# MoonInTheRiver/DiffSinger

Hardware: NVIDIA H100
Metric: mel-frames/s (higher is better)
Workload: dtype f16 operands (weights stochastically rounded per step), 1 MMA pass, conditioner projection hoisted (f32), f32 accumulate and state

## Files before the change

diffsinger_b200/csrc/dsx_hopper.cu:

```cuda
#include <stdio.h>
#include <string.h>

#include <algorithm>
#include <cmath>
#include <string>
#include <vector>

#include "dsx_internal.h"
#include "dsx_ptx.cuh"
#include "dsx_rng.cuh"

namespace dsx {

constexpr int kC = 256;
constexpr int kRowsPerLayer = 80 * 256;
constexpr int kSrRowsPerLayer = 32 * 256;
constexpr int kWBytes = 256 * 128;
constexpr int kABytes = 64 * 128;
constexpr int kZBytes = 4 * kABytes;
constexpr int kEpiBatch = 8;

constexpr int kHalo = 8;

template <int NWG, int R, bool WIN = (R == 3)>
struct StepCfg {
  static_assert(R == 2 || R == 3, "ring depth");
  static constexpr int THREADS = NWG * 128;
  static constexpr int STAGE = kWBytes + (WIN ? 0 : NWG * kABytes);
  static constexpr int BARS = R * STAGE;
  static constexpr int W = BARS + 1024;
  static constexpr int WROWS = 64 * NWG + 2 * kHalo;
  static constexpr int WBLK = WROWS * 128;
  static constexpr int ZHI23 = 2 * kABytes;
  static constexpr int ASLOT = NWG * ZHI23;
  static constexpr int WSIZE = WIN ? std::max(4 * WBLK, ASLOT + R * NWG * kABytes) : 0;
  static constexpr int ZHI = W + WSIZE;
  static constexpr int ZHI_WG = WIN ? 2 * kABytes : kZBytes;
  static constexpr int ZLO = ZHI + NWG * ZHI_WG;
  static constexpr int SMEM = 1024 + ZLO + NWG * (R == 2 ? kZBytes : kABytes);
  static_assert(WBLK % 1024 == 0 && ASLOT % 1024 == 0, "window blocks and activation slots start 1024-aligned");
  static_assert(!WIN || NWG * ZHI23 <= WSIZE, "z hi k-blocks 2-3 fit in W");
  static_assert(SMEM <= 232448, "shared memory budget (227 KB per block on sm_90)");
};
constexpr int kCondSmem = 1024 + StepCfg<2, 3, false>::BARS + 2 * 3 * 8;

struct HpParams {
  const __half* w;
  int w_sr;
  int P;
  int HP;
  int ylo;
  int fast_gate;
  const __half* whead;
  float* X;
  float* SKIP;
  __half* Y;
  __half* S16;
  const __half* CONDH;
  size_t plane;
  float* CP;
  const float* b1p;
  const float* b2;
  const float* dtab;
  int d_row_stride;
  int T, Tp, B, units;
  int l0, l1, L, cycle;
  float inv_sqrt_l;
  int head_flags;
  float* x;
  dsx_strides xs;
  float* eps;
  const float* noise;
  unsigned long long seed, offset;
  int b_off;
  DdpmCoef c;
  PlmsFuse pl;
  const float* bs;
  const float* bf;
  const float* bin;
  const float* d0;
  int d0_row_stride;
  int M;
  long long* trace;
  int trace_ctas;
  unsigned* flags;
};

__device__ __forceinline__ void stamp(const HpParams& p, int slot) {
  if (p.trace != nullptr && threadIdx.x == 0 && slot < DSX_TRACE_SLOTS && static_cast<int>(blockIdx.x) < p.trace_ctas) {
    long long t;
    asm volatile("mov.u64 %0, %%globaltimer;" : "=l"(t)::"memory");
    p.trace[static_cast<size_t>(blockIdx.x) * DSX_TRACE_SLOTS + slot] = t;
  }
}
__device__ __forceinline__ int layer_slot(const HpParams& p, int l, int k) { return 1 + 9 * (l - p.l0) + k; }
__device__ __forceinline__ int head_slot(const HpParams& p, int k) { return 1 + 9 * (p.l1 - p.l0) + k; }

template <int NWG>
__device__ __forceinline__ int partner_tile(const HpParams& p, int u) {
  if (p.units > static_cast<int>(gridDim.x) || p.B < 2) return -1;
  const int tpu = p.Tp / (64 * NWG), b = u / tpu;
  if (b & 1) return u - tpu;
  return b + 1 < p.B ? u + tpu : -1;
}

template <int NWG>
__device__ __forceinline__ void wait_neighbours(const HpParams& p, int u, unsigned n) {
  const int tpu = p.Tp / (64 * NWG);
  if (u % tpu != 0) wait_geq(p.flags + u - 1, n);
  if ((u + 1) % tpu != 0) wait_geq(p.flags + u + 1, n);
}

template <int NWG>
__device__ __forceinline__ void wait_layer(const HpParams& p, int l, int u) {
  if (threadIdx.x == 0) {
    const unsigned n = l - p.l0;
    if (n > 0) wait_neighbours<NWG>(p, u, n);
    const int pu = partner_tile<NWG>(p, u);
    if (pu >= 0 && pu < u) wait_geq(p.flags + p.units + pu, n + 1);
  }
  __syncthreads();
}

template <int NT>
__device__ __forceinline__ void load_w(uint8_t* dst, const __half* src0, const __half* src1, int nrows, int tid) {
  const uint32_t d = smem_u32(dst);
  for (int i = tid; i < nrows * 8; i += NT) {
    const int r = i >> 3, c = i & 7;
    const __half* src = (r < 128 ? src0 + static_cast<size_t>(r) * 64 : src1 + static_cast<size_t>(r - 128) * 64) + c * 8;
// ... 6 lines not shown
  for (int k = 0; k < 4; ++k) {
    const int i = wtid + k * 128;
    const int r = i >> 3, c = i & 7, t = t0 + r;
    const bool valid = t >= 0 && t < T;
    cp16(d + sw128(r, c), src + (static_cast<size_t>(b) * Tp + (valid ? t : 0)) * kC + ch0 + c * 8, valid);
  }
}
template <int NT>
__device__ __forceinline__ void load_wblock(uint8_t* dst, const __half* utt, int t_first, int ch0, int rows, int T, int tid) {
  const uint32_t d = smem_u32(dst);
#pragma unroll 1
  for (int i = tid; i < rows * 8; i += NT) {
    const int r = i >> 3, c = i & 7, t = t_first + r;
    const bool valid = t >= 0 && t < T;
    cp16_hint(d + sw128(r, c), utt + static_cast<size_t>(valid ? t : 0) * kC + ch0 + c * 8, valid, l2_evict_first());
  }
}

template <int N>
__device__ __forceinline__ void fence_acc(float (&d)[N]) {
#pragma unroll
  for (int i = 0; i < N; ++i) asm volatile("" : "+f"(d[i])::"memory");
}

struct NoPrefetch {
  __device__ __forceinline__ void operator()(int) const {}
};

__device__ __forceinline__ uint8_t* smem_base() {
  extern __shared__ uint8_t smem_raw[];
  return reinterpret_cast<uint8_t*>((reinterpret_cast<uintptr_t>(smem_raw) + 1023) & ~uintptr_t(1023));
}

template <int NWG, int R, bool WIN = (R == 3)>
struct Smem {
  using Cfg = StepCfg<NWG, R, WIN>;
  uint32_t n, nw;
  __device__ __forceinline__ uint8_t* slot(uint32_t i) const { return smem_base() + (i % R) * Cfg::STAGE; }
  __device__ __forceinline__ uint32_t full(uint32_t i) const { return smem_u32(smem_base() + Cfg::BARS) + (i % R) * 8; }
  __device__ __forceinline__ uint32_t empty(uint32_t i) const { return full(i) + R * 8; }
  __device__ __forceinline__ uint32_t parity(uint32_t i) const { return (i / R) & 1; }
  __device__ __forceinline__ uint8_t* wblk(int c) const { return smem_base() + Cfg::W + c * Cfg::WBLK; }
  __device__ __forceinline__ uint32_t wbar(int c) const { return full(0) + 2 * R * 8 + c * 8; }
  __device__ __forceinline__ uint8_t* ablk(int j, int wg) const {
    if (WIN) return smem_base() + Cfg::W + Cfg::ASLOT + j * NWG * kABytes + wg * kABytes;
    return smem_base() + j * Cfg::STAGE + kWBytes + wg * kABytes;
  }
  __device__ __forceinline__ uint8_t* zblk(int plane, int kb) const {
    const int wg = threadIdx.x >> 7;
    if (plane == 0) {
      if (WIN && kb >= 2) return smem_base() + Cfg::W + wg * Cfg::ZHI23 + (kb - 2) * kABytes;
      return smem_base() + Cfg::ZHI + wg * Cfg::ZHI_WG + kb * kABytes;
    }
    if (!WIN) return smem_base() + Cfg::ZLO + wg * kZBytes + kb * kABytes;
    return kb < R ? ablk(kb, wg) : smem_base() + Cfg::ZLO + wg * kABytes;
  }
  __device__ __forceinline__ uint8_t* zat(int plane, int r, int k) const {
    return zblk(plane, k >> 6) + sw128(r, (k & 63) >> 3) + (k & 7) * 2;
  }
  __device__ __forceinline__ void init() {
    n = 0;
    nw = 0;
    if (threadIdx.x == 0) {
      for (int j = 0; j < R; ++j) {
        mbar_init(full(j), 1 + NWG * 128);
        mbar_init(empty(j), NWG);
      }
      if (WIN)
        for (int c = 0; c < 4; ++c) mbar_init(wbar(c), NWG * 128);
      fence_mbar_init();
    }
    __syncthreads();
  }
};

enum PhaseKind { PH_NONE, PH_G1, PH_G2, PH_H1, PH_H2, PH_IN, PH_COND };
struct Phase {
  int kind, l, u, hq;
};
__device__ __forceinline__ Phase head_phase(const HpParams& p, int u) {
  const int kind = u >= p.units ? PH_NONE : (p.head_flags & TC_HEAD) ? PH_H1 : (p.head_flags & TC_INPROJ) ? PH_IN : PH_NONE;
  return Phase{kind, 0, u, 0};
}
__device__ __forceinline__ Phase after_layer(const HpParams& p, int l) {
  const int u0 = blockIdx.x;
  if (l + 1 < p.l1) return Phase{PH_G1, l + 1, u0, 0};
  return p.head_flags ? head_phase(p, u0) : Phase{PH_NONE, 0, 0, 0};
}

struct StageSrc {
  const __half* w0;
  const __half* w1;
  uint32_t wbytes;
  const __half* a;
  int b, at, ach;
  int wrow;
  int zplane, zkb;
};

__device__ __forceinline__ const __half* w1_tile(const HpParams& p, int l, int plane, int h, int kb) {
  if (p.w_sr) return p.w + (static_cast<size_t>(l) * kSrRowsPerLayer + (h * 12 + kb) * 256) * 64;
  return p.w + (static_cast<size_t>(l) * kRowsPerLayer + ((plane * 2 + h) * 16 + kb) * 256) * 64;
}
__device__ __forceinline__ const __half* w2_tile(const HpParams& p, int l, int plane, int q, int kb) {
  if (p.w_sr) return p.w + (static_cast<size_t>(l) * kSrRowsPerLayer + (24 + q * 4 + kb) * 256) * 64;
  return p.w + (static_cast<size_t>(l) * kRowsPerLayer + (64 + (plane * 2 + q) * 4 + kb) * 256) * 64;
}
__device__ __forceinline__ const __half* whead_tile(const HpParams& p, int idx) {
  return p.whead + static_cast<size_t>(idx) * 128 * 64;
}
__device__ __forceinline__ int pass_wplane(int ps) { return ps == 1 ? 1 : 0; }
__device__ __forceinline__ int pass_aplane(int ps) { return ps == 2 ? 1 : 0; }

__device__ __forceinline__ int phase_passes(const HpParams& p, int kind) {
  return kind == PH_COND ? 3 : (kind >= PH_H1 ? p.HP : p.P);
}
__device__ __forceinline__ int phase_stages(const HpParams& p, const Phase& ph) {
  const int kbs = ph.kind == PH_G1 ? 12 : ph.kind == PH_IN ? 2 : ph.kind == PH_NONE ? 0 : 4;
  return kbs * phase_passes(p, ph.kind);
}

template <int NWG, bool WIN>
__device__ __forceinline__ StageSrc stage_src(const HpParams& p, const Phase& ph, int s) {
  const int frame0 = ph.u * 64 * NWG;
  const int P = phase_passes(p, ph.kind);
  const int kb = s / P, ps = s % P, wp = pass_wplane(ps), ap = pass_aplane(ps);
  StageSrc st;
  st.w1 = nullptr;
  st.wbytes = kWBytes;
  st.a = nullptr;
  st.b = frame0 / p.Tp;
  st.at = frame0 % p.Tp + (threadIdx.x >> 7) * 64;
  st.ach = kb * 64;
  st.wrow = -1;
  st.zplane = ap;
  st.zkb = kb;
  switch (ph.kind) {
    case PH_G1: {
      const int shift = ((kb >> 2) - 1) * (1 << (ph.l % p.cycle));
      st.w0 = w1_tile(p, ph.l, wp, ph.hq, kb);
      st.ach = (kb & 3) * 64;
      if (WIN) {
        st.wrow = kHalo + (threadIdx.x >> 7) * 64 + shift;
      } else {
        st.a = p.Y + static_cast<size_t>(ph.l & 1) * 2 * p.plane + ap * p.plane;
        st.at += shift;
      }
      break;
    }
    case PH_G2:
      st.w0 = w2_tile(p, ph.l, wp, ph.hq, kb);
      break;
    case PH_H1:
      st.w0 = whead_tile(p, wp * 8 + kb);
      st.w1 = whead_tile(p, wp * 8 + 4 + kb);
      st.wbytes = kWBytes / 2;
      st.a = p.S16 + ap * p.plane;
      break;
    case PH_H2:
      st.w0 = whead_tile(p, 16 + wp * 4 + kb);
      st.wbytes = kWBytes / 2;
      break;
    case PH_IN:
      st.w0 = whead_tile(p, 24 + wp * 4 + kb);
      st.w1 = whead_tile(p, 24 + wp * 4 + 2 + kb);
      st.wbytes = kWBytes / 2;
      break;
    default:
      st.w0 = p.w + (static_cast<size_t>(ph.l) * kRowsPerLayer + ((wp * 2 + ph.hq) * 16 + 12 + kb) * 256) * 64;
      st.a = p.CONDH + ap * p.plane;
      break;
  }
  return st;
}

enum { kIssueW = 1, kIssueA = 2 };
template <int NWG, int R, bool WIN>
__device__ __forceinline__ void issue(const HpParams& p, const Smem<NWG, R, WIN>& sm, const StageSrc& st, uint32_t i,
                                      int parts) {
  const uint32_t full = sm.full(i);
  uint8_t* slot = sm.slot(i);
  if ((parts & kIssueW) && threadIdx.x == 0) {
    mbar_wait(sm.empty(i), sm.parity(i) ^ 1);
    mbar_arrive_expect_tx(full, st.w1 ? 2 * st.wbytes : st.wbytes);
    bulk_g2s(smem_u32(slot), st.w0, st.wbytes, full);
    if (st.w1) bulk_g2s(smem_u32(slot) + st.wbytes, st.w1, st.wbytes, full);
  }
  if (parts & kIssueA) {
    if (st.a) load_a(sm.ablk(i % R, threadIdx.x >> 7), st.a, st.b, st.at, st.ach, p.T, p.Tp, threadIdx.x & 127);
    if (WIN && !st.a) mbar_arrive(full);
    else cp_arrive_noinc(full);
  }
}

template <int NWG, int R, bool WIN>
__device__ __forceinline__ void load_window(const HpParams& p, const Smem<NWG, R, WIN>& sm, int l, int u) {
  const int frame0 = u * 64 * NWG;
  const __half* utt = p.Y + static_cast<size_t>(l & 1) * 2 * p.plane + static_cast<size_t>(frame0 / p.Tp) * p.Tp * kC;
#pragma unroll 1
  for (int c = 0; c < 4; ++c) {
    load_wblock<NWG * 128>(sm.wblk(c), utt, frame0 % p.Tp - kHalo, c * 64, StepCfg<NWG, R, WIN>::WROWS, p.T, threadIdx.x);
    cp_arrive_noinc(sm.wbar(c));
  }
}

template <int NWG, int R, bool WIN>
__device__ __forceinline__ void fill(const HpParams& p, const Smem<NWG, R, WIN>& sm, const Phase& ph, int parts) {
  if (WIN && ph.kind == PH_G1 && ph.hq == 0 && (parts & kIssueA)) load_window(p, sm, ph.l, ph.u);
  const int n = min(R, phase_stages(p, ph));
#pragma unroll 1
  for (int j = 0; j < n; ++j) issue(p, sm, stage_src<NWG, WIN>(p, ph, j), sm.n + j, parts);
}

template <int NH, int NWG, int R, bool WIN, class Pre = NoPrefetch>
__device__ __forceinline__ void gemm(float (&c0)[64], float (&c1)[64], Smem<NWG, R, WIN>& sm, const HpParams& p,
                                     const Phase& ph, Pre pre = Pre()) {
  const int nst = phase_stages(p, ph);
  const int wg = threadIdx.x >> 7;
  fence_proxy_async_smem();
  wg_bar_sync();
  fence_acc(c0);
  if (NH == 2) fence_acc(c1);
#pragma unroll 1
  for (int s = 0; s < nst; ++s) {
    const uint32_t i = sm.n + s;
    const StageSrc st = stage_src<NWG, WIN>(p, ph, s);
    mbar_wait(sm.full(i), sm.parity(i));
    if (WIN && st.wrow >= 0) mbar_wait(sm.wbar(st.ach >> 6), sm.nw & 1);
    fence_proxy_async_smem();
    uint8_t* slot = sm.slot(i);
    const uint8_t* aop = WIN && st.wrow >= 0 ? sm.wblk(st.ach >> 6) + st.wrow * 128
                         : st.a ? (WIN ? sm.ablk(i % R, wg) : slot + kWBytes + wg * kABytes)
                                : sm.zblk(st.zplane, st.zkb);
    const uint64_t a = wg_desc(smem_u32(aop));
    const uint64_t w = wg_desc(smem_u32(slot));
    wg_fence();
#pragma unroll
    for (int k4 = 0; k4 < 4; ++k4) {
      const int acc = (s > 0 || k4 > 0) ? 1 : 0;
      wgmma_n128(c0, a + 2 * k4, w + 2 * k4, acc);
      if (NH == 2) wgmma_n128(c1, a + 2 * k4, w + (16384 >> 4) + 2 * k4, acc);
    }
    wg_commit();
    if (s > 0) {
      wg_wait1();
      if ((threadIdx.x & 127) == 0) mbar_arrive(sm.empty(i - 1));
      if (s - 1 + R < nst) issue(p, sm, stage_src<NWG, WIN>(p, ph, s - 1 + R), i - 1 + R, kIssueW | kIssueA);
    }
    pre(s);
  }
  wg_wait0();
  fence_acc(c0);
  if (NH == 2) fence_acc(c1);
  if ((threadIdx.x & 127) == 0) mbar_arrive(sm.empty(sm.n + nst - 1));
  sm.n += nst;
}

template <int NWG, int R, bool WIN>
__device__ __forceinline__ void layer_tile(const HpParams& p, int l, int u, Smem<NWG, R, WIN>& sm) {
  const int tid = threadIdx.x, wg = tid >> 7, wtid = tid & 127;
  const int frame0 = u * 64 * NWG;
  const int b = frame0 / p.Tp, t0 = frame0 % p.Tp + wg * 64;
  const size_t fbase = static_cast<size_t>(b) * p.Tp + t0;
  const int P = p.P;
  const size_t NF = p.plane / kC;
  float c0[64], c1[64];

#pragma unroll 1
  for (int h = 0; h < 2; ++h) {
    auto pre = [&](int s) {
      if (wtid != 0 || s >= 8 || h != 0) return;
      prefetch_l2_hint(p.CP + (static_cast<size_t>(l) * NF + fbase) * 512 + s * 4096, 16384, l2_evict_last());
    };
    gemm<2>(c0, c1, sm, p, Phase{PH_G1, l, u, h}, pre);
    fill(p, sm, h == 0 ? Phase{PH_G1, l, u, 1} : Phase{PH_G2, l, u, 0}, kIssueW | kIssueA);
    if (WIN && h == 1) {
      sm.nw++;
      __syncthreads();
    }
    stamp(p, layer_slot(p, l, 2 * h));
    const float* cp = p.CP + (static_cast<size_t>(l) * NF + fbase) * 512 + h * 256;
#pragma unroll
    for (int e0 = 0; e0 < 64; e0 += 2 * kEpiBatch) {
      float2 cgv[kEpiBatch], cfv[kEpiBatch];
#pragma unroll
      for (int j = 0; j < kEpiBatch; ++j) {
        const int e = e0 + 2 * j, r = acc_row(wtid, e), n = acc_col(wtid, e);
        cgv[j] = ld_stream_f2(cp + static_cast<size_t>(r) * 512 + n);
        cfv[j] = ld_stream_f2(cp + static_cast<size_t>(r) * 512 + 128 + n);
      }
#pragma unroll
      for (int j = 0; j < kEpiBatch; ++j) {
        const int e = e0 + 2 * j, r = acc_row(wtid, e), n = acc_col(wtid, e);
        float z0, z1;
        if (p.fast_gate) {
          z0 = gate_fast(c0[e] + cgv[j].x, c1[e] + cfv[j].x);
          z1 = gate_fast(c0[e + 1] + cgv[j].y, c1[e + 1] + cfv[j].y);
        } else {
          z0 = gate_acc(c0[e] + cgv[j].x, c1[e] + cfv[j].x);
          z1 = gate_acc(c0[e + 1] + cgv[j].y, c1[e + 1] + cfv[j].y);
        }
        const __half2 hh = __floats2half2_rn(z0, z1);
        *reinterpret_cast<__half2*>(sm.zat(0, r, 128 * h + n)) = hh;
        if (R == 2 && P == 3) {
          const float2 hf = __half22float2(hh);
          *reinterpret_cast<__half2*>(sm.zat(1, r, 128 * h + n)) = __floats2half2_rn(z0 - hf.x, z1 - hf.y);
        }
      }
    }
    stamp(p, layer_slot(p, l, 2 * h + 1));
    if (h == 1 && tid == 0 && partner_tile<NWG>(p, u) > u) st_release_gpu(p.flags + p.units + u, l - p.l0 + 1);
  }

  const bool last = (l + 1 == p.L);
  const float* dnext = last ? nullptr : p.dtab + static_cast<size_t>(b) * p.d_row_stride + static_cast<size_t>(l + 1) * kC;
  __half* Yout = p.Y + static_cast<size_t>((l + 1) & 1) * 2 * p.plane;
#pragma unroll 1
  for (int q = 0; q < 2; ++q) {
    gemm<2>(c0, c1, sm, p, Phase{PH_G2, l, u, q});
    if (q == 0) fill(p, sm, Phase{PH_G2, l, u, 1}, kIssueW | kIssueA);
    else if (u + static_cast<int>(gridDim.x) < p.units) {
      const Phase next{PH_G1, l, u + static_cast<int>(gridDim.x), 0};
      fill(p, sm, next, kIssueW);
      wait_layer<NWG>(p, l, next.u);
      fill(p, sm, next, kIssueA);
    } else {
      fill(p, sm, after_layer(p, l), kIssueW);
    }
    stamp(p, layer_slot(p, l, 4 + 2 * q));
    const int row0 = acc_row(wtid, 0), colb = acc_col(wtid, 0);
    const bool ok0 = t0 + row0 < p.T, ok8 = t0 + row0 + 8 < p.T;
    const size_t tb = (fbase + row0) * kC + colb;
    const float* bias = p.b2 + static_cast<size_t>(l) * 512 + q * 256 + colb;
    const float* dn = last ? nullptr : dnext + colb;
    const float* src = (q == 0 ? p.X : p.SKIP) + tb;
    float* dst = (q == 0 ? p.X : p.SKIP) + tb;
    __half* yo = Yout + tb;
    __half* so = p.S16 + tb;
    const bool read_old = q == 0 || l > 0;
    const bool read_d = q == 0 && !last;
#pragma unroll
    for (int hh = 0; hh < 2; ++hh) {
#pragma unroll
      for (int e0 = 0; e0 < 64; e0 += 2 * kEpiBatch) {
        float2 old[kEpiBatch], bbv[kEpiBatch / 2], dvv[kEpiBatch / 2];
#pragma unroll
        for (int j = 0; j < kEpiBatch; ++j) {
          const int e = e0 + 2 * j, o = ((e & 2) ? 8 * kC : 0) + hh * 128 + (e >> 2) * 8;
          old[j] = make_float2(0.f, 0.f);
          if (read_old && ((e & 2) ? ok8 : ok0)) old[j] = *reinterpret_cast<const float2*>(src + o);
        }
#pragma unroll
        for (int i = 0; i < kEpiBatch / 2; ++i) {
          const int c = hh * 128 + ((e0 >> 2) + i) * 8;
          bbv[i] = __ldg(reinterpret_cast<const float2*>(bias + c));
          dvv[i] = make_float2(0.f, 0.f);
          if (read_d) dvv[i] = __ldg(reinterpret_cast<const float2*>(dn + c));
        }
#pragma unroll
        for (int j = 0; j < kEpiBatch; ++j) {
          const int e = e0 + 2 * j, c = hh * 128 + (e >> 2) * 8, o = ((e & 2) ? 8 * kC : 0) + c;
          if (!((e & 2) ? ok8 : ok0)) continue;
          const float a0 = hh ? c1[e] : c0[e], a1 = hh ? c1[e + 1] : c0[e + 1];
          const float2 bb = bbv[j >> 1];
          if (q == 0) {
            float2 xv = old[j];
            xv.x = (xv.x + (a0 + bb.x)) * 0.70710678118654752440f;
            xv.y = (xv.y + (a1 + bb.y)) * 0.70710678118654752440f;
            *reinterpret_cast<float2*>(dst + o) = xv;
            if (!last) {
              const float2 dv = dvv[j >> 1];
              const float ya = xv.x + dv.x, yb = xv.y + dv.y;
              const __half2 hy = __floats2half2_rn(ya, yb);
              *reinterpret_cast<__half2*>(yo + o) = hy;
              if (p.ylo) {
                const float2 hf = __half22float2(hy);
                *reinterpret_cast<__half2*>(yo + p.plane + o) = __floats2half2_rn(ya - hf.x, yb - hf.y);
              }
            }
          } else {
            float2 sk = make_float2(a0 + bb.x, a1 + bb.y);
            if (l > 0) {
              sk.x = old[j].x + sk.x;
              sk.y = old[j].y + sk.y;
            }
            *reinterpret_cast<float2*>(dst + o) = sk;
            if (last) {
              const float sa = sk.x * p.inv_sqrt_l, sb = sk.y * p.inv_sqrt_l;
              const __half2 hs = __floats2half2_rn(sa, sb);
              const float2 hf = __half22float2(hs);
              *reinterpret_cast<__half2*>(so + o) = hs;
              *reinterpret_cast<__half2*>(so + p.plane + o) = __floats2half2_rn(sa - hf.x, sb - hf.y);
            }
          }
        }
      }
    }
    stamp(p, layer_slot(p, l, 5 + 2 * q));
    if (q == 0) {
      __syncthreads();
      if (tid == 0) st_release_gpu(p.flags + u, l - p.l0 + 1);
    }
  }
}

template <int NWG, int R>
__device__ __forceinline__ void head_tile(const HpParams& p, int u, Smem<NWG, R>& sm) {
  const int tid = threadIdx.x, wg = tid >> 7, wtid = tid & 127;
  const int frame0 = u * 64 * NWG;
  const int b = frame0 / p.Tp, t0 = frame0 % p.Tp + wg * 64;
  const size_t fbase = static_cast<size_t>(b) * p.Tp + t0;
  const int flags = p.head_flags;
  const bool do_head = flags & TC_HEAD, do_in = flags & TC_INPROJ;
  float c0[64], c1[64];
#pragma unroll
  for (int i = 0; i < 64; ++i) c0[i] = 0.f;

  if (do_head) {
    gemm<2>(c0, c1, sm, p, Phase{PH_H1, 0, u, 0});
    fill(p, sm, Phase{PH_H2, 0, u, 0}, kIssueW | kIssueA);
    stamp(p, head_slot(p, 0));
#pragma unroll
    for (int hh = 0; hh < 2; ++hh) {
#pragma unroll
      for (int e = 0; e < 64; e += 2) {
        const int r = acc_row(wtid, e), col = hh * 128 + acc_col(wtid, e);
        const float2 bb = __ldg(reinterpret_cast<const float2*>(p.bs + col));
        const float a0 = fmaxf((hh ? c1[e] : c0[e]) + bb.x, 0.f), a1 = fmaxf((hh ? c1[e + 1] : c0[e + 1]) + bb.y, 0.f);
        const __half2 hv = __floats2half2_rn(a0, a1);
        *reinterpret_cast<__half2*>(sm.zat(0, r, col)) = hv;
        const float2 hf = __half22float2(hv);
        *reinterpret_cast<__half2*>(sm.zat(1, r, col)) = __floats2half2_rn(a0 - hf.x, a1 - hf.y);
      }
    }
    stamp(p, head_slot(p, 1));
    gemm<1>(c0, c1, sm, p, Phase{PH_H2, 0, u, 0});
    fill(p, sm, do_in ? Phase{PH_IN, 0, u, 0} : head_phase(p, u + gridDim.x), kIssueW | kIssueA);
    stamp(p, head_slot(p, 2));
  }

  const bool need_x = (flags & (TC_UPDATE | TC_INPROJ | TC_PLMS)) != 0;
  const bool need_z = (flags & TC_UPDATE) && p.c.sigma != 0.f;
#pragma unroll
  for (int e = 0; e < 64; e += 2) {
    const int r = acc_row(wtid, e), m = acc_col(wtid, e);
    const int t = t0 + r;
    const bool valid = t < p.T && m < p.M;
    float xv[2] = {0.f, 0.f};
    if (valid) {
      const size_t xrow = static_cast<size_t>(b) * p.xs.b + static_cast<size_t>(t) * p.xs.t;
      float zn[2] = {0.f, 0.f};
      if (need_x)
        for (int i = 0; i < 2; ++i) xv[i] = p.x[xrow + static_cast<size_t>(m + i) * p.xs.c];
      if (need_z) {
        if (p.noise) {
          for (int i = 0; i < 2; ++i) zn[i] = p.noise[(static_cast<size_t>(b) * p.M + m + i) * p.T + t];
        } else {
          const float4 z4 = philox_normal4(p.seed, p.offset, mel_noise_block(b + p.b_off, m, t, p.M, p.T));
          zn[0] = (m & 3) == 0 ? z4.x : z4.z;
          zn[1] = (m & 3) == 0 ? z4.y : z4.w;
        }
      }
#pragma unroll
      for (int i = 0; i < 2; ++i) {
        const int mm = m + i;
        const size_t ei = (static_cast<size_t>(b) * p.M + mm) * p.T + t;
        float ev = 0.f;
        if (do_head) ev = c0[e + i] + __ldg(p.bf + mm);
        if (flags & TC_WRITE_EPS) p.eps[ei] = ev;
// ... 38 lines not shown
  const float* d0 = p.d0 + static_cast<size_t>(b) * p.d0_row_stride;
#pragma unroll
  for (int hh = 0; hh < 2; ++hh) {
#pragma unroll
    for (int e = 0; e < 64; e += 2) {
      const int r = acc_row(wtid, e), col = hh * 128 + acc_col(wtid, e);
      if (t0 + r >= p.T) continue;
      const float2 bb = __ldg(reinterpret_cast<const float2*>(p.bin + col));
      const float2 dv = __ldg(reinterpret_cast<const float2*>(d0 + col));
      const float x0 = fmaxf((hh ? c1[e] : c0[e]) + bb.x, 0.f), x1 = fmaxf((hh ? c1[e + 1] : c0[e + 1]) + bb.y, 0.f);
      const size_t off = (fbase + r) * kC + col;
      *reinterpret_cast<float2*>(p.X + off) = make_float2(x0, x1);
      const float ya = x0 + dv.x, yb = x1 + dv.y;
      const __half2 hy = __floats2half2_rn(ya, yb);
      *reinterpret_cast<__half2*>(p.Y + off) = hy;
      if (p.ylo) {
        const float2 hf = __half22float2(hy);
        *reinterpret_cast<__half2*>(p.Y + p.plane + off) = __floats2half2_rn(ya - hf.x, yb - hf.y);
      }
    }
  }
  stamp(p, head_slot(p, 5));
}

template <int NWG, int R>
__global__ void __launch_bounds__(NWG * 128, 1) k_hp_step(const __grid_constant__ HpParams p) {
  Smem<NWG, R> sm;
  sm.init();
  stamp(p, 0);
  const int u0 = blockIdx.x;
  fill(p, sm, p.l0 < p.l1 ? Phase{PH_G1, p.l0, u0, 0} : head_phase(p, u0), kIssueW);
  for (int l = p.l0; l < p.l1; ++l) {
    wait_layer<NWG>(p, l, u0);
    if (l > p.l0) stamp(p, layer_slot(p, l - 1, 8));
    fill(p, sm, Phase{PH_G1, l, u0, 0}, kIssueA);
    for (int u = u0; u < p.units; u += gridDim.x) layer_tile<NWG, R>(p, l, u, sm);
  }
  if (p.head_flags) {
    __syncthreads();
    if (p.l0 < p.l1) stamp(p, layer_slot(p, p.l1 - 1, 8));
    fill(p, sm, head_phase(p, u0), kIssueA);
    for (int u = u0; u < p.units; u += gridDim.x) head_tile<NWG, R>(p, u, sm);
  }
}

__global__ void __launch_bounds__(256, 1) k_hp_condproj(const __grid_constant__ HpParams p) {
  Smem<2, 3, false> sm;
  sm.init();
  const int tid = threadIdx.x, wg = tid >> 7, wtid = tid & 127;
  const int u = blockIdx.x, l = blockIdx.y;
  const int frame0 = u * 128;
  const int b = frame0 / p.Tp, t0 = frame0 % p.Tp + wg * 64;
  const size_t fbase = static_cast<size_t>(b) * p.Tp + t0;
  const size_t NF = p.plane / kC;
  float c0[64], c1[64];
  fill(p, sm, Phase{PH_COND, l, u, 0}, kIssueW | kIssueA);
#pragma unroll 1
  for (int h = 0; h < 2; ++h) {
    gemm<2>(c0, c1, sm, p, Phase{PH_COND, l, u, h});
    if (h == 0) fill(p, sm, Phase{PH_COND, l, u, 1}, kIssueW | kIssueA);
    float* cp = p.CP + (static_cast<size_t>(l) * NF + fbase) * 512 + h * 256;
    const float* bias = p.b1p + (static_cast<size_t>(l) * 2 + h) * 256;
#pragma unroll
    for (int hh = 0; hh < 2; ++hh) {
#pragma unroll
      for (int e = 0; e < 64; e += 2) {
        const int r = acc_row(wtid, e), n = hh * 128 + acc_col(wtid, e);
        const float2 bb = __ldg(reinterpret_cast<const float2*>(bias + n));
        *reinterpret_cast<float2*>(cp + static_cast<size_t>(r) * 512 + n) =
            make_float2((hh ? c1[e] : c0[e]) + bb.x, (hh ? c1[e + 1] : c0[e + 1]) + bb.y);
      }
    }
  }
// ... 100 lines not shown
  DSX_CHECK(tc_supported(h), DSX_E_INVALID, "tensor-core path needs residual_channels == hidden_size == 256 (got %d, %d)",
            h->m.C, h->m.H);
  __half* wpack;
  float* b1p;
  const size_t rows = static_cast<size_t>(h->m.L) * kRowsPerLayer;
  DSX_TRY(h->mem.alloc(&wpack, rows * 64 * sizeof(__half)));
  DSX_TRY(h->mem.alloc(&b1p, static_cast<size_t>(h->m.L) * 512 * sizeof(float)));
  k_pack_wtc<<<dim3(kRowsPerLayer / 256, h->m.L), 256, 0, s>>>(h->m.w1f, h->m.w2f, h->m.b1f, wpack, b1p);
  DSX_TRY(counted_launch(h, "k_pack_wtc"));
  h->m.wpack = wpack;
  h->m.b1p = b1p;
  __half* whead;
  DSX_TRY(h->mem.alloc(&whead, static_cast<size_t>(32) * 128 * 64 * sizeof(__half)));
  k_pack_whead<<<32, 128, 0, s>>>(h->m.skip_w, h->m.fin_w, h->m.in_w, whead, h->m.M);
  DSX_TRY(counted_launch(h, "k_pack_whead"));
  h->m.whead = whead;
  h->m.wsr = nullptr;
  h->m.wsr_sets = 0;
  if (h->precision == DSX_PREC_FP16S) {
    const int R = std::max(1, h->sr_sets);
    __half* wsr;
    const size_t srows = static_cast<size_t>(R) * h->m.L * kSrRowsPerLayer;
    DSX_TRY(h->mem.alloc(&wsr, srows * 64 * sizeof(__half)));
    k_pack_wsr<<<dim3(32, h->m.L, R), 256, 0, s>>>(h->m.w1f, h->m.w2f, wsr, h->m.L, h->sr_seed);
    DSX_TRY(counted_launch(h, "k_pack_wsr"));
    h->m.wsr = wsr;
    h->m.wsr_sets = R;
  }
  return DSX_OK;
}

template <int NWG, int R>
static int step_capacity(dsx_handle* h) {
  int& cache = h->step_occ[NWG == 1 ? 0 : R == 3 ? 1 : 2];
  if (cache == 0) {
    using Cfg = StepCfg<NWG, R>;
    cudaFuncSetAttribute(k_hp_step<NWG, R>, cudaFuncAttributeMaxDynamicSharedMemorySize, Cfg::SMEM);
    int n = 0;
    cudaError_t e = cudaOccupancyMaxActiveBlocksPerMultiprocessor(&n, k_hp_step<NWG, R>, Cfg::THREADS, Cfg::SMEM);
    if (e != cudaSuccess) cudaGetLastError();
    cache = (e == cudaSuccess && n >= 1) ? n * h->sm_count : -1;
  }
  return cache;
}

static HpParams base_params(dsx_handle* h, const Geom& g, int rows) {
  const ModelDev& m = h->m;
  HpParams prm;
  memset(&prm, 0, sizeof(prm));
  prm.whead = m.whead;
  prm.X = h->ws.X;
  prm.SKIP = h->ws.SKIP;
  prm.Y = h->ws.Y;
  prm.S16 = h->ws.S16;
  prm.CONDH = h->ws.CONDH;
  prm.plane = g.frames_padded() * kC;
  prm.CP = h->ws.CP;
  prm.b1p = m.b1p;
  prm.b2 = m.b2f;
  prm.T = g.T; prm.Tp = g.Tp; prm.B = g.B;
  prm.units = static_cast<int>(g.frames_padded() / rows);
  prm.L = m.L; prm.cycle = m.cycle;
  prm.inv_sqrt_l = 1.0f / sqrtf(static_cast<float>(m.L));
  prm.HP = (h->precision == DSX_PREC_FP16) ? 1 : 3;
  prm.ylo = (h->precision == DSX_PREC_FP16X3) ? 1 : 0;
  prm.M = m.M;
  prm.bs = m.skip_b;
// ... 313 lines not shown
```

diffsinger_b200/csrc/dsx_ptx.cuh:

```cuda
#pragma once
#include <cuda_fp16.h>
#include <stdint.h>

namespace dsx {

__device__ __forceinline__ uint32_t smem_u32(const void* p) {
  return static_cast<uint32_t>(__cvta_generic_to_shared(p));
}

__device__ __forceinline__ uint32_t sw128(int r, int c) { return static_cast<uint32_t>(r * 128 + ((c ^ (r & 7)) << 4)); }
__host__ __device__ __forceinline__ int sw128_elem(int r, int k) { return r * 64 + ((((k >> 3) ^ r) & 7) << 3) + (k & 7); }

__device__ __forceinline__ uint64_t wg_desc(uint32_t smem_addr) {
  return static_cast<uint64_t>((smem_addr & 0x3FFFF) >> 4) | (static_cast<uint64_t>(1) << 16) |
         (static_cast<uint64_t>(1024 >> 4) << 32) | (static_cast<uint64_t>(1) << 62);
}

__device__ __forceinline__ void wg_fence() { asm volatile("wgmma.fence.sync.aligned;" ::: "memory"); }
__device__ __forceinline__ void wg_commit() { asm volatile("wgmma.commit_group.sync.aligned;" ::: "memory"); }
__device__ __forceinline__ void wg_wait0() { asm volatile("wgmma.wait_group.sync.aligned 0;" ::: "memory"); }
__device__ __forceinline__ void wg_wait1() { asm volatile("wgmma.wait_group.sync.aligned 1;" ::: "memory"); }
__device__ __forceinline__ void wg_bar_sync() {
  if (threadIdx.x < 128) asm volatile("bar.sync 1, 128;" ::: "memory");
  else asm volatile("bar.sync 2, 128;" ::: "memory");
// ... 76 lines not shown
        "+f"(d[41]), "+f"(d[42]), "+f"(d[43]), "+f"(d[44]), "+f"(d[45]), "+f"(d[46]), "+f"(d[47]), "+f"(d[48]),
        "+f"(d[49]), "+f"(d[50]), "+f"(d[51]), "+f"(d[52]), "+f"(d[53]), "+f"(d[54]), "+f"(d[55]), "+f"(d[56]),
        "+f"(d[57]), "+f"(d[58]), "+f"(d[59]), "+f"(d[60]), "+f"(d[61]), "+f"(d[62]), "+f"(d[63])
      : "l"(da), "l"(db), "r"(accumulate)
      : "memory");
}

template <int N>
__device__ __forceinline__ void wgmma_f16_bmn(float (&d)[N / 2], uint64_t da, uint64_t db, int accumulate);
template <>
__device__ __forceinline__ void wgmma_f16_bmn<64>(float (&d)[32], uint64_t da, uint64_t db, int accumulate) {
  asm volatile(
      "{\n\t.reg .pred p;\n\tsetp.ne.b32 p, %34, 0;\n\t"
      "wgmma.mma_async.sync.aligned.m64n64k16.f32.f16.f16 "
      "{%0, %1, %2, %3, %4, %5, %6, %7, %8, %9, %10, %11, %12, %13, %14, %15, %16, %17, %18, %19, %20, %21, %22, %23, %24, %25, %26, %27, %28, %29, %30, %31}, %32, %33, p, 1, 1, 0, 1;\n\t}"
      : "+f"(d[0]), "+f"(d[1]), "+f"(d[2]), "+f"(d[3]), "+f"(d[4]), "+f"(d[5]), "+f"(d[6]), "+f"(d[7]), "+f"(d[8]), "+f"(d[9]), "+f"(d[10]), "+f"(d[11]), "+f"(d[12]), "+f"(d[13]), "+f"(d[14]), "+f"(d[15]), "+f"(d[16]), "+f"(d[17]), "+f"(d[18]), "+f"(d[19]), "+f"(d[20]), "+f"(d[21]), "+f"(d[22]), "+f"(d[23]), "+f"(d[24]), "+f"(d[25]), "+f"(d[26]), "+f"(d[27]), "+f"(d[28]), "+f"(d[29]), "+f"(d[30]), "+f"(d[31])
      : "l"(da), "l"(db), "r"(accumulate)
      : "memory");
}
template <>
__device__ __forceinline__ void wgmma_f16_bmn<128>(float (&d)[64], uint64_t da, uint64_t db, int accumulate) {
  asm volatile(
      "{\n\t.reg .pred p;\n\tsetp.ne.b32 p, %66, 0;\n\t"
      "wgmma.mma_async.sync.aligned.m64n128k16.f32.f16.f16 "
      "{%0, %1, %2, %3, %4, %5, %6, %7, %8, %9, %10, %11, %12, %13, %14, %15, %16, %17, %18, %19, %20, %21, %22, %23, %24, %25, %26, %27, %28, %29, %30, %31, %32, %33, %34, %35, %36, %37, %38, %39, %40, %41, %42, %43, %44, %45, %46, %47, %48, %49, %50, %51, %52, %53, %54, %55, %56, %57, %58, %59, %60, %61, %62, %63}, %64, %65, p, 1, 1, 0, 1;\n\t}"
      : "+f"(d[0]), "+f"(d[1]), "+f"(d[2]), "+f"(d[3]), "+f"(d[4]), "+f"(d[5]), "+f"(d[6]), "+f"(d[7]), "+f"(d[8]), "+f"(d[9]), "+f"(d[10]), "+f"(d[11]), "+f"(d[12]), "+f"(d[13]), "+f"(d[14]), "+f"(d[15]), "+f"(d[16]), "+f"(d[17]), "+f"(d[18]), "+f"(d[19]), "+f"(d[20]), "+f"(d[21]), "+f"(d[22]), "+f"(d[23]), "+f"(d[24]), "+f"(d[25]), "+f"(d[26]), "+f"(d[27]), "+f"(d[28]), "+f"(d[29]), "+f"(d[30]), "+f"(d[31]), "+f"(d[32]), "+f"(d[33]), "+f"(d[34]), "+f"(d[35]), "+f"(d[36]), "+f"(d[37]), "+f"(d[38]), "+f"(d[39]), "+f"(d[40]), "+f"(d[41]), "+f"(d[42]), "+f"(d[43]), "+f"(d[44]), "+f"(d[45]), "+f"(d[46]), "+f"(d[47]), "+f"(d[48]), "+f"(d[49]), "+f"(d[50]), "+f"(d[51]), "+f"(d[52]), "+f"(d[53]), "+f"(d[54]), "+f"(d[55]), "+f"(d[56]), "+f"(d[57]), "+f"(d[58]), "+f"(d[59]), "+f"(d[60]), "+f"(d[61]), "+f"(d[62]), "+f"(d[63])
      : "l"(da), "l"(db), "r"(accumulate)
      : "memory");
}

__device__ __forceinline__ int acc_row(int wtid, int e) { return ((wtid >> 5) << 4) + ((wtid & 31) >> 2) + ((e & 2) ? 8 : 0); }
__device__ __forceinline__ int acc_col(int wtid, int e) { return ((e >> 2) << 3) + ((wtid & 3) << 1) + (e & 1); }

__device__ __forceinline__ void cp16(uint32_t dst, const void* src, bool valid) {
  asm volatile("cp.async.cg.shared.global [%0], [%1], 16, %2;" ::"r"(dst), "l"(src), "r"(valid ? 16 : 0) : "memory");
}
__device__ __forceinline__ void cp16_hint(uint32_t dst, const void* src, bool valid, uint64_t pol) {
  asm volatile("cp.async.cg.shared.global.L2::cache_hint [%0], [%1], 16, %2, %3;" ::"r"(dst), "l"(src),
               "r"(valid ? 16 : 0), "l"(pol)
               : "memory");
}
__device__ __forceinline__ void cp_commit() { asm volatile("cp.async.commit_group;" ::: "memory"); }
template <int N>
__device__ __forceinline__ void cp_wait() { asm volatile("cp.async.wait_group %0;" ::"n"(N) : "memory"); }

__device__ __forceinline__ void mbar_init(uint32_t bar, uint32_t count) {
  asm volatile("mbarrier.init.shared::cta.b64 [%0], %1;" ::"r"(bar), "r"(count) : "memory");
}
__device__ __forceinline__ void fence_mbar_init() { asm volatile("fence.mbarrier_init.release.cluster;" ::: "memory"); }
__device__ __forceinline__ void mbar_wait(uint32_t bar, uint32_t parity) {
  asm volatile(
      "{\n\t.reg .pred p;\n"
      "WAIT:\n\t"
      "mbarrier.try_wait.parity.shared::cta.b64 p, [%0], %1;\n\t"
      "@!p bra WAIT;\n\t}" ::"r"(bar),
      "r"(parity)
      : "memory");
}
__device__ __forceinline__ void mbar_arrive(uint32_t bar) {
  asm volatile("mbarrier.arrive.shared::cta.b64 _, [%0];" ::"r"(bar) : "memory");
}
__device__ __forceinline__ void mbar_arrive_expect_tx(uint32_t bar, uint32_t bytes) {
  asm volatile("mbarrier.arrive.expect_tx.shared::cta.b64 _, [%0], %1;" ::"r"(bar), "r"(bytes) : "memory");
}
__device__ __forceinline__ void cp_arrive_noinc(uint32_t bar) {
  asm volatile("cp.async.mbarrier.arrive.noinc.shared::cta.b64 [%0];" ::"r"(bar) : "memory");
// ... 69 lines not shown
```

Baseline: 95760.

## Feed second-GEMM activations from registers via register-A WGMMA in windowed path

In the windowed (R=3) configuration, the gated activation z is packed into f16 register fragments and consumed directly by a register-sourced m64n128k16 WGMMA, so it is no longer written to shared memory. The second GEMM is split into four half-width (128-column) groups, each loading two half-weight tiles per stage, and the epilogue handles one column half at a time. This removes the z shared-memory planes and the post-G1 __syncthreads, which shrinks shared memory and may allow more resident blocks. The cost is 64 more live registers, more GEMM and fill rounds per layer, and a changed ring-buffer schedule. The head GEMM uses the same register-A path.

Result: faster. 98290, median of 6 (+2.6%).

```diff
diff --git a/diffsinger_b200/csrc/dsx_hopper.cu b/diffsinger_b200/csrc/dsx_hopper.cu
--- a/diffsinger_b200/csrc/dsx_hopper.cu
+++ b/diffsinger_b200/csrc/dsx_hopper.cu
@@ -22,7 +22,7 @@
 
 constexpr int kHalo = 8;
 
-template <int NWG, int R, bool WIN = (R == 3)>
+template <int NWG, int R, bool WIN = (R != 2)>
 struct StepCfg {
   static_assert(R == 2 || R == 3, "ring depth");
   static constexpr int THREADS = NWG * 128;
@@ -31,15 +31,12 @@
   static constexpr int W = BARS + 1024;
   static constexpr int WROWS = 64 * NWG + 2 * kHalo;
   static constexpr int WBLK = WROWS * 128;
-  static constexpr int ZHI23 = 2 * kABytes;
-  static constexpr int ASLOT = NWG * ZHI23;
-  static constexpr int WSIZE = WIN ? std::max(4 * WBLK, ASLOT + R * NWG * kABytes) : 0;
+  static constexpr int HEADBLKS = 4;
+  static constexpr int WSIZE = WIN ? std::max(4 * WBLK, HEADBLKS * NWG * kABytes) : 0;
   static constexpr int ZHI = W + WSIZE;
-  static constexpr int ZHI_WG = WIN ? 2 * kABytes : kZBytes;
-  static constexpr int ZLO = ZHI + NWG * ZHI_WG;
-  static constexpr int SMEM = 1024 + ZLO + NWG * (R == 2 ? kZBytes : kABytes);
-  static_assert(WBLK % 1024 == 0 && ASLOT % 1024 == 0, "window blocks and activation slots start 1024-aligned");
-  static_assert(!WIN || NWG * ZHI23 <= WSIZE, "z hi k-blocks 2-3 fit in W");
+  static constexpr int ZLO = ZHI + NWG * kZBytes;
+  static constexpr int SMEM = 1024 + (WIN ? ZHI : R == 2 ? ZLO + NWG * kZBytes : W);
+  static_assert(WBLK % 1024 == 0, "window blocks start 1024-aligned");
   static_assert(SMEM <= 232448, "shared memory budget (227 KB per block on sm_90)");
 };
 constexpr int kCondSmem = 1024 + StepCfg<2, 3, false>::BARS + 2 * 3 * 8;
@@ -93,8 +90,18 @@
     p.trace[static_cast<size_t>(blockIdx.x) * DSX_TRACE_SLOTS + slot] = t;
   }
 }
-__device__ __forceinline__ int layer_slot(const HpParams& p, int l, int k) { return 1 + 9 * (l - p.l0) + k; }
-__device__ __forceinline__ int head_slot(const HpParams& p, int k) { return 1 + 9 * (p.l1 - p.l0) + k; }
+__device__ __forceinline__ void stamp_extend(const HpParams& p, int slot, int since) {
+  if (p.trace != nullptr && threadIdx.x == 0 && slot < DSX_TRACE_SLOTS && since < DSX_TRACE_SLOTS &&
+      static_cast<int>(blockIdx.x) < p.trace_ctas) {
+    long long t;
+    asm volatile("mov.u64 %0, %%globaltimer;" : "=l"(t)::"memory");
+    long long* row = p.trace + static_cast<size_t>(blockIdx.x) * DSX_TRACE_SLOTS;
+    row[slot] += t - row[since];
+  }
+}
+constexpr int kLayerSlots = 9;
+__device__ __forceinline__ int layer_slot(const HpParams& p, int l, int k) { return 1 + kLayerSlots * (l - p.l0) + k; }
+__device__ __forceinline__ int head_slot(const HpParams& p, int k) { return 1 + kLayerSlots * (p.l1 - p.l0) + k; }
 
 template <int NWG>
 __device__ __forceinline__ int partner_tile(const HpParams& p, int u) {
@@ -167,7 +174,7 @@
   return reinterpret_cast<uint8_t*>((reinterpret_cast<uintptr_t>(smem_raw) + 1023) & ~uintptr_t(1023));
 }
 
-template <int NWG, int R, bool WIN = (R == 3)>
+template <int NWG, int R, bool WIN = (R != 2)>
 struct Smem {
   using Cfg = StepCfg<NWG, R, WIN>;
   uint32_t n, nw;
@@ -178,17 +185,13 @@
   __device__ __forceinline__ uint8_t* wblk(int c) const { return smem_base() + Cfg::W + c * Cfg::WBLK; }
   __device__ __forceinline__ uint32_t wbar(int c) const { return full(0) + 2 * R * 8 + c * 8; }
   __device__ __forceinline__ uint8_t* ablk(int j, int wg) const {
-    if (WIN) return smem_base() + Cfg::W + Cfg::ASLOT + j * NWG * kABytes + wg * kABytes;
+    if (WIN) return smem_base() + Cfg::W + j * NWG * kABytes + wg * kABytes;
     return smem_base() + j * Cfg::STAGE + kWBytes + wg * kABytes;
   }
   __device__ __forceinline__ uint8_t* zblk(int plane, int kb) const {
     const int wg = threadIdx.x >> 7;
-    if (plane == 0) {
-      if (WIN && kb >= 2) return smem_base() + Cfg::W + wg * Cfg::ZHI23 + (kb - 2) * kABytes;
-      return smem_base() + Cfg::ZHI + wg * Cfg::ZHI_WG + kb * kABytes;
-    }
-    if (!WIN) return smem_base() + Cfg::ZLO + wg * kZBytes + kb * kABytes;
-    return kb < R ? ablk(kb, wg) : smem_base() + Cfg::ZLO + wg * kABytes;
+    if (WIN) return ablk(plane == 0 ? 2 + kb : kb, wg);
+    return smem_base() + (plane == 0 ? Cfg::ZHI : Cfg::ZLO) + wg * kZBytes + kb * kABytes;
   }
   __device__ __forceinline__ uint8_t* zat(int plane, int r, int k) const {
     return zblk(plane, k >> 6) + sw128(r, (k & 63) >> 3) + (k & 7) * 2;
@@ -250,9 +253,10 @@
 __device__ __forceinline__ int phase_passes(const HpParams& p, int kind) {
   return kind == PH_COND ? 3 : (kind >= PH_H1 ? p.HP : p.P);
 }
+template <bool WIN>
 __device__ __forceinline__ int phase_stages(const HpParams& p, const Phase& ph) {
   const int kbs = ph.kind == PH_G1 ? 12 : ph.kind == PH_IN ? 2 : ph.kind == PH_NONE ? 0 : 4;
-  return kbs * phase_passes(p, ph.kind);
+  return kbs * phase_passes(p, ph.kind) / (WIN && ph.kind == PH_G2 ? 2 : 1);
 }
 
 template <int NWG, bool WIN>
@@ -284,7 +288,14 @@
       break;
     }
     case PH_G2:
-      st.w0 = w2_tile(p, ph.l, wp, ph.hq, kb);
+      if (WIN) {
+        const int t0 = 2 * s, t1 = 2 * s + 1, rows = (ph.hq & 1) * 128 * 64;
+        st.w0 = w2_tile(p, ph.l, pass_wplane(t0 % P), ph.hq >> 1, t0 / P) + rows;
+        st.w1 = w2_tile(p, ph.l, pass_wplane(t1 % P), ph.hq >> 1, t1 / P) + rows;
+        st.wbytes = kWBytes / 2;
+      } else {
+        st.w0 = w2_tile(p, ph.l, wp, ph.hq, kb);
+      }
       break;
     case PH_H1:
       st.w0 = whead_tile(p, wp * 8 + kb);
@@ -342,7 +353,7 @@
 template <int NWG, int R, bool WIN>
 __device__ __forceinline__ void fill(const HpParams& p, const Smem<NWG, R, WIN>& sm, const Phase& ph, int parts) {
   if (WIN && ph.kind == PH_G1 && ph.hq == 0 && (parts & kIssueA)) load_window(p, sm, ph.l, ph.u);
-  const int n = min(R, phase_stages(p, ph));
+  const int n = min(R, phase_stages<WIN>(p, ph));
 #pragma unroll 1
   for (int j = 0; j < n; ++j) issue(p, sm, stage_src<NWG, WIN>(p, ph, j), sm.n + j, parts);
 }
@@ -350,7 +361,7 @@
 template <int NH, int NWG, int R, bool WIN, class Pre = NoPrefetch>
 __device__ __forceinline__ void gemm(float (&c0)[64], float (&c1)[64], Smem<NWG, R, WIN>& sm, const HpParams& p,
                                      const Phase& ph, Pre pre = Pre()) {
-  const int nst = phase_stages(p, ph);
+  const int nst = phase_stages<WIN>(p, ph);
   const int wg = threadIdx.x >> 7;
   fence_proxy_async_smem();
   wg_bar_sync();
@@ -391,6 +402,47 @@
   sm.n += nst;
 }
 
+template <int SUB, int PS, int NWG, int R>
+__device__ __forceinline__ void gemm_ra(float (&c)[64], const uint32_t (&zr)[64], Smem<NWG, R, true>& sm,
+                                        const HpParams& p, const Phase& ph) {
+  constexpr int nst = 4 * PS / SUB;
+  fence_proxy_async_smem();
+  wg_bar_sync();
+  fence_acc(c);
+#pragma unroll
+  for (int s = 0; s < nst; ++s) {
+    const uint32_t i = sm.n + s;
+    mbar_wait(sm.full(i), sm.parity(i));
+    const uint64_t w = wg_desc(smem_u32(sm.slot(i)));
+    wg_fence();
+#pragma unroll
+    for (int j = 0; j < SUB; ++j) {
+      const int t = s * SUB + j, kb = t / PS;
+#pragma unroll
+      for (int k4 = 0; k4 < 4; ++k4) {
+        const int acc = (t > 0 || k4 > 0) ? 1 : 0;
+        const uint64_t wd = w + j * (16384 >> 4) + 2 * k4;
+        if (pass_aplane(t % PS) == 0) {
+          const int r = 16 * kb + 4 * k4;
+          wgmma_n128_ra(c, zr[r], zr[r + 1], zr[r + 2], zr[r + 3], wd, acc);
+        } else {
+          wgmma_n128(c, wg_desc(smem_u32(sm.zblk(1, kb))) + 2 * k4, wd, acc);
+        }
+      }
+    }
+    wg_commit();
+    if (s > 0) {
+      wg_wait1();
+      if ((threadIdx.x & 127) == 0) mbar_arrive(sm.empty(i - 1));
+      if (s - 1 + R < nst) issue(p, sm, stage_src<NWG, true>(p, ph, s - 1 + R), i - 1 + R, kIssueW | kIssueA);
+    }
+  }
+  wg_wait0();
+  fence_acc(c);
+  if ((threadIdx.x & 127) == 0) mbar_arrive(sm.empty(sm.n + nst - 1));
+  sm.n += nst;
+}
+
 template <int NWG, int R, bool WIN>
 __device__ __forceinline__ void layer_tile(const HpParams& p, int l, int u, Smem<NWG, R, WIN>& sm) {
   const int tid = threadIdx.x, wg = tid >> 7, wtid = tid & 127;
@@ -400,8 +452,9 @@
   const int P = p.P;
   const size_t NF = p.plane / kC;
   float c0[64], c1[64];
-
-#pragma unroll 1
+  uint32_t zr[64];
+
+#pragma unroll(WIN ? 2 : 1)
   for (int h = 0; h < 2; ++h) {
     auto pre = [&](int s) {
       if (wtid != 0 || s >= 8 || h != 0) return;
@@ -409,10 +462,7 @@
     };
     gemm<2>(c0, c1, sm, p, Phase{PH_G1, l, u, h}, pre);
     fill(p, sm, h == 0 ? Phase{PH_G1, l, u, 1} : Phase{PH_G2, l, u, 0}, kIssueW | kIssueA);
-    if (WIN && h == 1) {
-      sm.nw++;
-      __syncthreads();
-    }
+    if (WIN && h == 1) sm.nw++;
     stamp(p, layer_slot(p, l, 2 * h));
     const float* cp = p.CP + (static_cast<size_t>(l) * NF + fbase) * 512 + h * 256;
 #pragma unroll
@@ -435,11 +485,15 @@
           z0 = gate_acc(c0[e] + cgv[j].x, c1[e] + cfv[j].x);
           z1 = gate_acc(c0[e + 1] + cgv[j].y, c1[e + 1] + cfv[j].y);
         }
-        const __half2 hh = __floats2half2_rn(z0, z1);
-        *reinterpret_cast<__half2*>(sm.zat(0, r, 128 * h + n)) = hh;
-        if (R == 2 && P == 3) {
-          const float2 hf = __half22float2(hh);
-          *reinterpret_cast<__half2*>(sm.zat(1, r, 128 * h + n)) = __floats2half2_rn(z0 - hf.x, z1 - hf.y);
+        if constexpr (WIN) {
+          zr[32 * h + e / 2] = a_pair(z0, z1);
+        } else {
+          const __half2 hh = __floats2half2_rn(z0, z1);
+          *reinterpret_cast<__half2*>(sm.zat(0, r, 128 * h + n)) = hh;
+          if (P == 3) {
+            const float2 hf = __half22float2(hh);
+            *reinterpret_cast<__half2*>(sm.zat(1, r, 128 * h + n)) = __floats2half2_rn(z0 - hf.x, z1 - hf.y);
+          }
         }
       }
     }
@@ -450,10 +504,17 @@
   const bool last = (l + 1 == p.L);
   const float* dnext = last ? nullptr : p.dtab + static_cast<size_t>(b) * p.d_row_stride + static_cast<size_t>(l + 1) * kC;
   __half* Yout = p.Y + static_cast<size_t>((l + 1) & 1) * 2 * p.plane;
+  constexpr int NG = WIN ? 4 : 2;
 #pragma unroll 1
-  for (int q = 0; q < 2; ++q) {
-    gemm<2>(c0, c1, sm, p, Phase{PH_G2, l, u, q});
-    if (q == 0) fill(p, sm, Phase{PH_G2, l, u, 1}, kIssueW | kIssueA);
+  for (int g = 0; g < NG; ++g) {
+    const int q = WIN ? g >> 1 : g;
+    if constexpr (WIN) {
+      if (P == 1) gemm_ra<2, 1>(c0, zr, sm, p, Phase{PH_G2, l, u, g});
+      else gemm_ra<2, 2>(c0, zr, sm, p, Phase{PH_G2, l, u, g});
+    } else {
+      gemm<2>(c0, c1, sm, p, Phase{PH_G2, l, u, g});
+    }
+    if (g + 1 < NG) fill(p, sm, Phase{PH_G2, l, u, g + 1}, kIssueW | kIssueA);
     else if (u + static_cast<int>(gridDim.x) < p.units) {
       const Phase next{PH_G1, l, u + static_cast<int>(gridDim.x), 0};
       fill(p, sm, next, kIssueW);
@@ -462,8 +523,9 @@
     } else {
       fill(p, sm, after_layer(p, l), kIssueW);
     }
-    stamp(p, layer_slot(p, l, 4 + 2 * q));
-    const int row0 = acc_row(wtid, 0), colb = acc_col(wtid, 0);
+    if (WIN && (g & 1)) stamp_extend(p, layer_slot(p, l, 4 + 2 * q), layer_slot(p, l, 5 + 2 * q));
+    else stamp(p, layer_slot(p, l, 4 + 2 * q));
+    const int row0 = acc_row(wtid, 0), colb = acc_col(wtid, 0) + (WIN ? (g & 1) * 128 : 0);
     const bool ok0 = t0 + row0 < p.T, ok8 = t0 + row0 + 8 < p.T;
     const size_t tb = (fbase + row0) * kC + colb;
     const float* bias = p.b2 + static_cast<size_t>(l) * 512 + q * 256 + colb;
@@ -475,7 +537,7 @@
     const bool read_old = q == 0 || l > 0;
     const bool read_d = q == 0 && !last;
 #pragma unroll
-    for (int hh = 0; hh < 2; ++hh) {
+    for (int hh = 0; hh < (WIN ? 1 : 2); ++hh) {
 #pragma unroll
       for (int e0 = 0; e0 < 64; e0 += 2 * kEpiBatch) {
         float2 old[kEpiBatch], bbv[kEpiBatch / 2], dvv[kEpiBatch / 2];
@@ -532,15 +594,15 @@
       }
     }
     stamp(p, layer_slot(p, l, 5 + 2 * q));
-    if (q == 0) {
+    if (g == NG / 2 - 1) {
       __syncthreads();
       if (tid == 0) st_release_gpu(p.flags + u, l - p.l0 + 1);
     }
   }
 }
 
-template <int NWG, int R>
-__device__ __forceinline__ void head_tile(const HpParams& p, int u, Smem<NWG, R>& sm) {
+template <int NWG, int R, bool WIN = (R != 2)>
+__device__ __forceinline__ void head_tile(const HpParams& p, int u, Smem<NWG, R, WIN>& sm) {
   const int tid = threadIdx.x, wg = tid >> 7, wtid = tid & 127;
   const int frame0 = u * 64 * NWG;
   const int b = frame0 / p.Tp, t0 = frame0 % p.Tp + wg * 64;
@@ -552,6 +614,7 @@
   for (int i = 0; i < 64; ++i) c0[i] = 0.f;
 
   if (do_head) {
+    uint32_t hr[64];
     gemm<2>(c0, c1, sm, p, Phase{PH_H1, 0, u, 0});
     fill(p, sm, Phase{PH_H2, 0, u, 0}, kIssueW | kIssueA);
     stamp(p, head_slot(p, 0));
@@ -563,13 +626,19 @@
         const float2 bb = __ldg(reinterpret_cast<const float2*>(p.bs + col));
         const float a0 = fmaxf((hh ? c1[e] : c0[e]) + bb.x, 0.f), a1 = fmaxf((hh ? c1[e + 1] : c0[e + 1]) + bb.y, 0.f);
         const __half2 hv = __floats2half2_rn(a0, a1);
-        *reinterpret_cast<__half2*>(sm.zat(0, r, col)) = hv;
+        if constexpr (WIN) hr[32 * hh + e / 2] = a_pair(a0, a1);
+        else *reinterpret_cast<__half2*>(sm.zat(0, r, col)) = hv;
         const float2 hf = __half22float2(hv);
         *reinterpret_cast<__half2*>(sm.zat(1, r, col)) = __floats2half2_rn(a0 - hf.x, a1 - hf.y);
       }
     }
     stamp(p, head_slot(p, 1));
-    gemm<1>(c0, c1, sm, p, Phase{PH_H2, 0, u, 0});
+    if constexpr (WIN) {
+      if (p.HP == 1) gemm_ra<1, 1>(c0, hr, sm, p, Phase{PH_H2, 0, u, 0});
+      else gemm_ra<1, 3>(c0, hr, sm, p, Phase{PH_H2, 0, u, 0});
+    } else {
+      gemm<1>(c0, c1, sm, p, Phase{PH_H2, 0, u, 0});
+    }
     fill(p, sm, do_in ? Phase{PH_IN, 0, u, 0} : head_phase(p, u + gridDim.x), kIssueW | kIssueA);
     stamp(p, head_slot(p, 2));
   }
@@ -674,13 +743,13 @@
   fill(p, sm, p.l0 < p.l1 ? Phase{PH_G1, p.l0, u0, 0} : head_phase(p, u0), kIssueW);
   for (int l = p.l0; l < p.l1; ++l) {
     wait_layer<NWG>(p, l, u0);
-    if (l > p.l0) stamp(p, layer_slot(p, l - 1, 8));
+    if (l > p.l0) stamp(p, layer_slot(p, l - 1, kLayerSlots - 1));
     fill(p, sm, Phase{PH_G1, l, u0, 0}, kIssueA);
     for (int u = u0; u < p.units; u += gridDim.x) layer_tile<NWG, R>(p, l, u, sm);
   }
   if (p.head_flags) {
     __syncthreads();
-    if (p.l0 < p.l1) stamp(p, layer_slot(p, p.l1 - 1, 8));
+    if (p.l0 < p.l1) stamp(p, layer_slot(p, p.l1 - 1, kLayerSlots - 1));
     fill(p, sm, head_phase(p, u0), kIssueA);
     for (int u = u0; u < p.units; u += gridDim.x) head_tile<NWG, R>(p, u, sm);
   }
@@ -847,7 +916,7 @@
 
 template <int NWG, int R>
 static int step_capacity(dsx_handle* h) {
-  int& cache = h->step_occ[NWG == 1 ? 0 : R == 3 ? 1 : 2];
+  int& cache = h->step_occ[R == 2 ? 2 : NWG - 1];
   if (cache == 0) {
     using Cfg = StepCfg<NWG, R>;
     cudaFuncSetAttribute(k_hp_step<NWG, R>, cudaFuncAttributeMaxDynamicSharedMemorySize, Cfg::SMEM);
diff --git a/diffsinger_b200/csrc/dsx_ptx.cuh b/diffsinger_b200/csrc/dsx_ptx.cuh
--- a/diffsinger_b200/csrc/dsx_ptx.cuh
+++ b/diffsinger_b200/csrc/dsx_ptx.cuh
@@ -132,6 +132,32 @@
 __device__ __forceinline__ int acc_row(int wtid, int e) { return ((wtid >> 5) << 4) + ((wtid & 31) >> 2) + ((e & 2) ? 8 : 0); }
 __device__ __forceinline__ int acc_col(int wtid, int e) { return ((e >> 2) << 3) + ((wtid & 3) << 1) + (e & 1); }
 
+__device__ __forceinline__ uint32_t a_pair(float v0, float v1) {
+  const __half2 h = __floats2half2_rn(v0, v1);
+  return *reinterpret_cast<const uint32_t*>(&h);
+}
+
+__device__ __forceinline__ void wgmma_n128_ra(float (&d)[64], uint32_t a0, uint32_t a1, uint32_t a2, uint32_t a3,
+                                              uint64_t db, int accumulate) {
+  asm volatile(
+      "{\n\t.reg .pred p;\n\tsetp.ne.b32 p, %69, 0;\n\t"
+      "wgmma.mma_async.sync.aligned.m64n128k16.f32.f16.f16 "
+      "{%0, %1, %2, %3, %4, %5, %6, %7, %8, %9, %10, %11, %12, %13, %14, %15, %16, %17, %18, %19, %20, %21, %22, %23, "
+      "%24, %25, %26, %27, %28, %29, %30, %31, %32, %33, %34, %35, %36, %37, %38, %39, %40, %41, %42, %43, %44, %45, %46, "
+      "%47, %48, %49, %50, %51, %52, %53, %54, %55, %56, %57, %58, %59, %60, %61, %62, %63}, {%64, %65, %66, %67}, %68, "
+      "p, 1, 1, 0;\n\t}"
+      : "+f"(d[0]), "+f"(d[1]), "+f"(d[2]), "+f"(d[3]), "+f"(d[4]), "+f"(d[5]), "+f"(d[6]), "+f"(d[7]), "+f"(d[8]),
+        "+f"(d[9]), "+f"(d[10]), "+f"(d[11]), "+f"(d[12]), "+f"(d[13]), "+f"(d[14]), "+f"(d[15]), "+f"(d[16]),
+        "+f"(d[17]), "+f"(d[18]), "+f"(d[19]), "+f"(d[20]), "+f"(d[21]), "+f"(d[22]), "+f"(d[23]), "+f"(d[24]),
+        "+f"(d[25]), "+f"(d[26]), "+f"(d[27]), "+f"(d[28]), "+f"(d[29]), "+f"(d[30]), "+f"(d[31]), "+f"(d[32]),
+        "+f"(d[33]), "+f"(d[34]), "+f"(d[35]), "+f"(d[36]), "+f"(d[37]), "+f"(d[38]), "+f"(d[39]), "+f"(d[40]),
+        "+f"(d[41]), "+f"(d[42]), "+f"(d[43]), "+f"(d[44]), "+f"(d[45]), "+f"(d[46]), "+f"(d[47]), "+f"(d[48]),
+        "+f"(d[49]), "+f"(d[50]), "+f"(d[51]), "+f"(d[52]), "+f"(d[53]), "+f"(d[54]), "+f"(d[55]), "+f"(d[56]),
+        "+f"(d[57]), "+f"(d[58]), "+f"(d[59]), "+f"(d[60]), "+f"(d[61]), "+f"(d[62]), "+f"(d[63])
+      : "r"(a0), "r"(a1), "r"(a2), "r"(a3), "l"(db), "r"(accumulate)
+      : "memory");
+}
+
 __device__ __forceinline__ void cp16(uint32_t dst, const void* src, bool valid) {
   asm volatile("cp.async.cg.shared.global [%0], [%1], 16, %2;" ::"r"(dst), "l"(src), "r"(valid ? 16 : 0) : "memory");
 }
```
